# Mikubill/sketch2img

Hardware: AMD Instinct MI355X
Metric: sketch-guided images/sec whole-node, SD1.5 512px 50-step DDIM (higher is better)
Workload: dtype fp16

## Files before the change

### include/skg.h

```cpp
#ifndef SKG_H_
#define SKG_H_

#include <stddef.h>
#include <stdint.h>

#ifdef __cplusplus
extern "C" {
#endif

#define SKG_OK 0
#define SKG_E_BADARG (-1)
#define SKG_E_UNSUPPORTED (-2)
#define SKG_E_LAUNCH (-3)

#define SKG_ABI_VERSION 6
int skg_abi_version(void);
const char* skg_last_error(void);

#define SKG_EPI_RELU 1u
#define SKG_EPI_OUT_F32 2u
#define SKG_EPI_GEGLU 4u
#define SKG_EPI_BIAS_ROWS 8u

int skg_gemm_f16(const void* A, int lda, const void* B, int ldb, void* C, void* C_lo, int ldc, int M, int N, int K,
// ... 25 lines not shown
int skg_gemm_f16_rows(const void* A, int lda, const void* B, int ldb, void* C, int ldc, int M, int N, int K,
                      const void* bias, int seg_rows, int seg_stride, void* stream);
int skg_conv3x3_up2_f16(const void* X, int ldx, const void* Wpp, void* Y, void* Y_lo, int ldy, int rows, int IH, int IW, int Cin,
                        int Cout, int pair_in, const void* bias, void* stream);
int skg_conv3x3_sc_f16(const void* X, int ldx, const void* X2, int ldx2, int K2, const void* Wcat, void* Y, void* Y_lo, int ldy,
                       int rows, int IH, int IW, int Cin, int Cout, const void* bias, unsigned flags, float* gn_partial, int groups,
                       void* stream);
size_t skg_conv3x3_wino_v_bytes(int rows, int IH, int IW, int Cin);
int skg_conv3x3_wino_f16(const void* X, int ldx, const void* U, void* V, void* Y, void* Y_lo, int ldy, int rows, int IH, int IW,
                         int Cin, int Cout, const void* bias, const void* residual, const void* residual_lo, int ldr, unsigned flags,
                         void* stream);
int skg_groupnorm_wino_fwd(const void* X, int ldx, void* V, int rows, int IH, int IW, int C, int groups, float eps,
                           const void* gamma, const void* beta, int silu, float* stats, void* stream);
int skg_conv4x4s2_f16(const void* X, int ldx, const void* W16, void* Y, int ldy, int rows, int IH, int IW, int Cin,
                      int Cout, const void* bias, void* stream);


int skg_groupnorm_apply(const void* X, const void* X_lo, int ldx, void* Y, int ldy, int rows, int HW, int C, int groups,
                        const float* stats, const void* gamma, const void* beta, int silu, void* stream);
int skg_groupnorm_bwd(const void* X, int ldx, const void* dY, int lddy, void* dX, int lddx,
                      const void* residual, int ldr, int rows, int HW, int C, int groups,
                      const float* stats, const void* gamma, const void* beta, int silu,
                      float* partial, void* stream);

int skg_layernorm_fwd(const void* X, const void* X_lo, int ldx, void* Y, int ldy, int M, int C, const void* gamma,
                      const void* beta, float eps, float* stats, void* stream);
int skg_layernorm_bwd(const void* X, int ldx, const void* dY, int lddy, void* dX, int lddx,
                      const void* residual, int ldr, int M, int C, const void* gamma,
                      const float* stats, void* stream);

// ... 150 lines not shown
```

### sketch2img_amd/_lib.py

```python
from __future__ import annotations

import ctypes
import os

import torch

_HERE = os.path.dirname(os.path.abspath(__file__))
LIB_PATH = os.environ.get("SKG_LIB") or os.path.join(_HERE, "libskg.so")

ABI_VERSION = 6

SIGNATURES = {
    "skg_abi_version": ("i", ""),
    "skg_last_error": ("s", ""),
    "skg_gemm_f16": ("i", "pipippiiiipppifupiip"),
    "skg_conv3x3_up2_f16": ("i", "pipppiiiiiiipp"),
    "skg_conv3x3_sc_f16": ("i", "pipiipppiiiiiipupip"),
    "skg_conv4x4s2_f16": ("i", "pippiiiiiipp"),
    "skg_conv3x3_wino_v_bytes": ("z", "iiii"),
    "skg_conv3x3_wino_f16": ("i", "pippppiiiiiipppiup"),
    "skg_groupnorm_wino_fwd": ("i", "pipiiiiifppipp"),
    "skg_gemm_f16_rows": ("i", "pipipiiiipiip"),
    "skg_gemm_gn_fused": ("i", "iiiiiii"),
    "skg_gemm_f16_geglu_keep": ("i", "pipipipiiiipp"),
    "skg_ff_block_f16": ("i", "ppippiiiippfppppppippiipiip"),
    "skg_xattn_block_f16": ("i", "ppippiiiiiippfpppfpppipip"),
    "skg_gemm_variant": ("i", "iiiii"),
    "skg_set_workspace": ("i", "pzp"),
    "skg_conv3x3_f16": ("i", "pipppiiiiiiipppifupip"),
    "skg_groupnorm_scratch_floats": ("z", "ii"),
    "skg_groupnorm_stats": ("i", "piiiiifppp"),
    "skg_groupnorm_fwd": ("i", "ppippiiiiifppippp"),
    "skg_groupnorm_from_partial": ("i", "ppippiiiiiifppippipiip"),
# ... 105 lines not shown
```

### sketch2img_amd/csrc/gemm.hip

```cpp
#include "gemm_params.h"
#include <mutex>
#include <vector>

namespace {

constexpr int BM = 128;
constexpr int BK = 32;
constexpr int PITCH = 40;

template <int BN, int MODE>
__global__ __launch_bounds__(256) void gemm_kernel(const GemmParams p) {
  constexpr int WN = BN / 2;
  constexpr int NT = WN / 16;
  constexpr int MT = 4;
  constexpr int BPT = BN / 64;
  __shared__ __attribute__((aligned(16))) half_t As[2][BM * PITCH];
  __shared__ __attribute__((aligned(16))) half_t Bs[2][BN * PITCH];

  const int tid = threadIdx.x;
  const int lane = tid & 63;
  const int wave = tid >> 6;
  const int wm = wave >> 1, wn = wave & 1;
  const int g = lane >> 4, l16 = lane & 15;
  const int m0 = blockIdx.y * BM;
// ... 463 lines not shown
              skg_aligned(Y, 16) && (!bias || skg_aligned(bias, 8)));
  hipStream_t st = (hipStream_t)stream;
  GemmParams p{};
  p.A = (const half_t*)X; p.lda = ldx;
  p.B = (const half_t*)W16; p.ldb = 16 * Cin;
  p.C = Y; p.ldc = ldy; p.bias = (const half_t*)bias;
  p.N = Cout; p.K = 16 * Cin; p.alpha = 1.f; p.flags = 0;
  p.IH = IH; p.IW = IW; p.OH = IH / 2; p.OW = IW / 2; p.Cin = Cin; p.M = rows * p.OH * p.OW;
  p.ntaps = 16;
  ws_attach(p, st);
  if (!skg_gemm2_try_launch(p, MODE_S2, st)) return SKG_E_UNSUPPORTED;
  SKG_CHECK_LAUNCH("skg_conv4x4s2_f16");
  return SKG_OK;
}

static void conv_out_size(int mode, int IH, int IW, int* OH, int* OW) {
  const int up = (mode == SKG_CONV_UP2 || mode == SKG_CONV_S2T), dn = (mode == SKG_CONV_S2 || mode == SKG_CONV_S2A);
  *OH = up ? IH * 2 : dn ? IH / 2 : IH;
  *OW = up ? IW * 2 : dn ? IW / 2 : IW;
}

extern "C" int skg_conv3x3_f16(const void* X, int ldx, const void* Wp, void* Y, void* Y_lo, int ldy, int rows, int IH, int IW,
                               int Cin, int Cout, int mode, const void* bias, const void* residual, const void* residual_lo,
                               int ldr, float alpha, unsigned flags, float* gn_partial, int groups, void* stream) {
  int OH, OW;
  conv_out_size(mode, IH, IW, &OH, &OW);
  SKG_REQUIRE(!(flags & SKG_EPI_BIAS_ROWS) || bias);
  SKG_REQUIRE(!(Y_lo || residual_lo) || pair_args_ok(Y, Y_lo, ldy, residual, residual_lo, ldr, Cin, flags));
  SKG_REQUIRE(!gn_partial || (rows > 0 && OH > 0 && OW > 0 && skg_aligned(Y, 16) &&
                              gn_args_ok(gn_partial, rows * OH * OW, Cout, OH * OW, groups, ldy, flags)));
// ... 30 lines not shown
```

### sketch2img_amd/csrc/gemm2.hip

```cpp
#include "gemm_params.h"
#include <stdlib.h>

namespace {

constexpr int BK = 64;
constexpr unsigned OOB = 0x80000000u;

typedef __attribute__((address_space(3))) void* lds_ptr_t;

__device__ __forceinline__ void dma16(__amdgpu_buffer_rsrc_t rsrc, half_t* lds_wave_base, unsigned voff,
                                      unsigned soff) {
  __builtin_amdgcn_raw_ptr_buffer_load_lds(rsrc, (lds_ptr_t)lds_wave_base, 16, voff, soff, 0, 0);
}

template <int MASK, int N>
__device__ __forceinline__ void sgb() {
  if constexpr (N > 0) __builtin_amdgcn_sched_group_barrier(MASK, N, 0);
}
constexpr int SGB_MFMA = 0x008, SGB_VMEM = 0x010, SGB_DSREAD = 0x100;
template <int NT, int R, int V>
__device__ __forceinline__ void sched_group() {
  if constexpr (NT > 0) {
    sgb<SGB_MFMA, 1>();
    if constexpr (R > 0) {
// ... 95 lines not shown
}

template <int BM, int BN, int WGM, int WGN, int MODE, int NS, bool GNS, bool HILO, bool FIX, bool BROWS = false>
__device__ __forceinline__ void gemm2_body(const GemmParams& p, int tiles_n, int nwg, unsigned a_bytes, unsigned b_bytes,
                                           unsigned a_shift, int kt_per_split, float* __restrict__ ws) {
  constexpr int NW = WGM * WGN;
  constexpr int NTHR = NW * 64;
  constexpr int WM = BM / WGM;
  constexpr int WN = BN / WGN;
  constexpr int NT = WN / 16;
  constexpr int MT = WM / 16;
  constexpr int ACH = BM / 8 / NW;
  constexpr int BCH = BN / 8 / NW;
  static_assert(BM % (8 * NW) == 0 && BN % (8 * NW) == 0 && WM % 16 == 0 && WN % 16 == 0, "tile shape");
  constexpr int STAGE = (BM + BN) * BK;
  constexpr bool AFFINE = (MODE == MODE_DIRECT || MODE == MODE_S1 || MODE == MODE_S2 || MODE == MODE_S2A);
  __shared__ __attribute__((aligned(16))) half_t smem[NS * STAGE + 2 * BN];

  const int tid = threadIdx.x;
  const int lane = tid & 63;
  const int wave = __builtin_amdgcn_readfirstlane(tid >> 6);
  const int wm = wave / WGN, wn = wave - wm * WGN;
  const int g = lane >> 4, l16 = lane & 15;

  const __amdgpu_buffer_rsrc_t rA =
      __builtin_amdgcn_make_buffer_rsrc((void*)((const char*)p.A - a_shift), 0, a_bytes, 0x00020000);
  const __amdgpu_buffer_rsrc_t rB = __builtin_amdgcn_make_buffer_rsrc((void*)p.B, 0, b_bytes, 0x00020000);
  const __amdgpu_buffer_rsrc_t rA2 = __builtin_amdgcn_make_buffer_rsrc(
      (void*)(p.A2 ? p.A2 : p.A), 0, p.A2 ? ((unsigned)(p.M - 1) * (unsigned)p.lda2 + (unsigned)p.K2) * 2u : 0u, 0x00020000);
  const int KT1 = (MODE == MODE_S1 && p.K2) ? (p.K - p.K2) / BK : (1 << 30);

// ... 6 lines not shown
    g_phase[vb][7] = __builtin_amdgcn_s_getreg((31 << 11) | 20);
    g_phase[vb][5] = __builtin_amdgcn_s_getreg((31 << 11) | 6);
  }
#endif
  int lid;
  {
    const int bid = vb;
    const int xcd = bid & 7, idx = bid >> 3;
    const int q = nwg >> 3, r = nwg & 7;
    lid = (xcd < r ? xcd * (q + 1) : r * (q + 1) + (xcd - r) * q) + idx;
  }
  const int ntiles = ws ? nwg / ((p.K / BK + kt_per_split - 1) / kt_per_split) : nwg;
  const int split = lid / ntiles;
  lid -= split * ntiles;
  int ph = p.up2 ? p.up2 - 1 : 0;
  if (p.up2 == 5) {
    const int per = ntiles >> 2;
    ph = lid / per;
    lid -= ph * per;
  }
  int tile_m = lid / tiles_n;
  int tile_n = lid - tile_m * tiles_n;
  if (const int gn = (p.flags >> 20) & 0xf) {
    const int G = ((p.flags >> 24) & 0xf) ? (int)((p.flags >> 24) & 0xf) : 8;
    const int per = ntiles / G, tmb = (ntiles / tiles_n) / (G / gn), tnb = tiles_n / gn;
    const int xr = lid / per, r = lid - xr * per;
    const int xm = xr / gn, xn = xr - xm * gn;
    const int rm = r / tnb;
    tile_m = xm * tmb + rm;
    tile_n = xn * tnb + (r - rm * tnb);
  }
  const int m0 = tile_m * BM, n0 = tile_n * BN;

  const int lr = lane >> 3;
  const int lq = lane & 7;
// ... 7 lines not shown
    const int r = (j * NW + wave) * 8 + lr;
    const unsigned pk = (unsigned)(lq ^ ((r >> 1) & 7)) * 16u;
    const int m = m0 + r;
    const bool ok = m < p.M;
    const int mm = ok ? m : 0;
    a_mask[j] = 0; a_oy[j] = a_ox[j] = 0; a_img[j] = 0;
    if (MODE == MODE_DIRECT) {
      a_voff[j] = ok ? (unsigned)mm * (unsigned)p.lda * 2u + pk : OOB;
    } else {
      const int ohw = p.OH * p.OW;
      const int b = mm / ohw;
      if (j == 0) smp0 = b;
      const int rr = mm - b * ohw;
      const int oy = rr / p.OW, ox = rr - oy * p.OW;
      const unsigned img = (unsigned)b * (unsigned)(p.IH * p.IW);
      if (MODE == MODE_S1 || MODE == MODE_S2 || MODE == MODE_S2A) {
        const int cy = MODE == MODE_S1 ? oy : 2 * oy + (MODE == MODE_S2A), cx = MODE == MODE_S1 ? ox : 2 * ox + (MODE == MODE_S2A);
        a_voff[j] = ok ? ((img + (unsigned)(cy * p.IW + cx)) * (unsigned)p.lda) * 2u + pk : OOB;
        unsigned mk = 0;
        if (MODE == MODE_S2 && p.ntaps == 16) {
#pragma unroll
          for (int t = 0; t < 16; ++t) {
            const int iy = cy + (t >> 2) - 1, ix = cx + (t & 3) - 1;
            if (ok && iy >= 0 && iy < p.IH && ix >= 0 && ix < p.IW) mk |= 1u << t;
          }
        } else {
#pragma unroll
          for (int t = 0; t < 9; ++t) {
            const int iy = cy + t / 3 - 1, ix = cx + t % 3 - 1;
            if (ok && iy >= 0 && iy < p.IH && ix >= 0 && ix < p.IW) mk |= 1u << t;
          }
        }
// ... 28 lines not shown
        d.va[j] = (live && m0 + r < p.M) ? (unsigned)(m0 + r) * (unsigned)p.lda2 * 2u + pk : OOB;
      }
#pragma unroll
      for (int j = 0; j < BCH; ++j) d.vb[j] = live ? b_voff[j] : OOB;
      d.soa = (unsigned)(kt - KT1) * (BK * 2u);
      d.sob = (unsigned)kt * (BK * 2u);
      return d;
    }
    const int k0 = kt * BK;
    unsigned soff = (unsigned)k0 * 2u;
    int tap = 0, ky = 0, kx = 0, c0 = 0;
    unsigned kb = (unsigned)k0;
    if (MODE != MODE_DIRECT) {
      int ti;
      if (tap_minor) {
        const int nt = p.ntaps ? p.ntaps : 9;
        const int cb = kt / nt;
        ti = kt - cb * nt;
        c0 = cb * BK;
      } else {
        ti = k0 / p.Cin;
        c0 = k0 - ti * p.Cin;
      }
      kb = (unsigned)(ti * p.Cin + c0);
      if (MODE == MODE_S2 && p.ntaps == 16) {
        tap = ti;
        ky = ti >> 2;
        kx = ti & 3;
      } else {
        const unsigned tapmap = p.up2 == 5 ? (unsigned)((ph >> 1) * 3 + (ph & 1)) * 0x1111u + 0x4310u : p.tapmap;
        tap = p.ntaps ? (int)((tapmap >> (4 * ti)) & 0xfu) : ti;
        ky = tap / 3;
        kx = tap - ky * 3;
      }
      const int ca = (p.a_wrap && c0 >= p.a_wrap) ? c0 - p.a_wrap : c0;
      soff = (unsigned)((ky * p.IW + kx) * p.lda + ca) * 2u;
    }
#pragma unroll
    for (int j = 0; j < ACH; ++j) {
      unsigned v;
// ... 108 lines not shown
    }
#endif
#pragma unroll
    for (int ks = 0; ks < 2; ++ks)
#pragma unroll
      for (int i = 0; i < MT; ++i)
#pragma unroll
        for (int j = 0; j < NT; ++j)
          acc[i][j] = __builtin_amdgcn_mfma_f32_16x16x32_f16(wf[ks][j], xf[ks][i], acc[i][j], 0, 0, 0);
#ifdef SKG_LAB
    if (!(p.flags & 0x2000u))
#endif
    sched_plan<MT, NT, ND>();
  };

  const int kt_begin = split * kt_per_split;
  const int KT = min(p.K / BK, kt_begin + kt_per_split);
  float bias_r = 0.f;
  if constexpr (!BROWS) {
    const half_t* bias_t = p.bias;
    if constexpr (MODE != MODE_DIRECT) bias_t += __builtin_amdgcn_readfirstlane(smp0) * p.bias_pitch;
    bias_r = (tid < BN && p.bias && n0 + tid < p.N) ? (float)bias_t[n0 + tid] : 0.f;
  }
  SKG_PH(1);
  {
    const DmaStep d0 = dma_prepare(kt_begin, true);
#pragma unroll
    for (int i = 0; i < ND; ++i) dma_one(d0, 0, i);
  }
  if constexpr (NS == 2) {
    for (int kt = kt_begin; kt < KT; kt += 2) {
      asm volatile("s_waitcnt vmcnt(0)" ::: "memory");
// ... 24 lines not shown
        }
      }
    }
  }
  asm volatile("s_waitcnt vmcnt(0)" ::: "memory");

  SKG_PH(2);
#ifdef SKG_PHASES
  if ((tid & 63) == 0 && vb < (1 << 15)) g_phase[vb][12 + (tid >> 6)] = __builtin_readcyclecounter();
#endif
  const bool stream_out = p.flags & 0x800u;
  const bool relu = p.flags & SKG_EPI_RELU;
  const bool f32out = p.flags & SKG_EPI_OUT_F32;
  if (ws) {
    float* slab = ws + (size_t)split * p.M * p.N;
#pragma unroll
    for (int i = 0; i < MT; ++i) {
      const int m = m0 + wm * WM + i * 16 + l16;
      if (m >= p.M) continue;
#pragma unroll
      for (int j = 0; j < NT; ++j) {
        const int n = n0 + wn * WN + j * 16 + g * 4;
        if (n < p.N) {
          *reinterpret_cast<float4_t*>(slab + (size_t)m * p.N + n) = acc[i][j];
        }
      }
    }
    if constexpr (FIX) {
      __shared__ unsigned s_ticket;
      const int splits = nwg / ntiles;
// ... 448 lines not shown
#endif

__global__ __launch_bounds__(256) void splitk_reduce_kernel(const GemmParams p, const float* __restrict__ ws,
                                                            int splits) {
  const int N4 = p.N >> 2;
  const size_t total = (size_t)p.M * N4;
  const size_t slab = (size_t)p.M * p.N;
  for (size_t i = (size_t)blockIdx.x * 256 + threadIdx.x; i < total; i += (size_t)gridDim.x * 256) {
    const size_t m = i / N4;
    const int n = (int)(i - m * N4) * 4;
    float4_t v = *reinterpret_cast<const float4_t*>(ws + m * p.N + n);
    for (int s = 1; s < splits; ++s) v += *reinterpret_cast<const float4_t*>(ws + s * slab + m * p.N + n);
    splitk_epilogue(p, v, m, n);
  }
}


struct SplitTuning { int target, smax, ns; };
inline SplitTuning read_split_tuning() {
  auto geti = [](const char* n, int dflt) { const char* e = getenv(n); return e ? atoi(e) : dflt; };
  SplitTuning t{geti("SKG_SPLIT_TARGET", 512), geti("SKG_MAX_SPLITS", 8), geti("SKG_SPLIT_NS", 3 )};
  t.target = t.target < 1 ? 1 : t.target > 4096 ? 4096 : t.target;
  t.smax = t.smax < 1 ? 1 : t.smax > 64 ? 64 : t.smax;
  t.ns = t.ns <= 2 ? 2 : t.ns >= 4 ? 4 : 3;
  return t;
}
inline SplitTuning split_tuning() {
#ifdef SKG_LAB
  return read_split_tuning();
#else
// ... 64 lines not shown
  if (!p.gn_partial || p.gn_groups <= 0 || p.gn_hw <= 0 || !eligible(p, mode)) return false;
  if (p.flags & (SKG_EPI_OUT_F32 | SKG_EPI_GEGLU)) return false;
  const bool hilo = p.c_lo || p.res_lo;
  TileCfg t = pick_tile(p.M, p.N, p.K);
  if (hilo && t.bm == 256) t = TileCfg{128, 160};
  if (t.bm != 128 || t.bn != 160) return false;
  if (p.M % 128 != 0 || p.N % 160 != 0 || p.gn_hw % 128 != 0 || p.M % p.gn_hw != 0 || p.N % p.gn_groups != 0) return false;
  const int cpg = p.N / p.gn_groups;
  if ((cpg & 1) || 160 % cpg != 0) return false;
  if (p.ldc % 8 != 0 || (reinterpret_cast<uintptr_t>(p.C) & 15) != 0) return false;
  if (p.res && (p.ldr % 8 != 0 || (reinterpret_cast<uintptr_t>(p.res) & 15) != 0)) return false;
  const long ntiles = (long)(p.M / 128) * (p.N / 160);
  return pick_splits(ntiles, p.K / BK, (size_t)p.M * p.N * 4, p.ws, p.ws_bytes) == 1;
}

template <int BM, int BN, int WGM, int WGN, int MODE>
void launch_cfg(const GemmParams& p_in, hipStream_t st) {
  GemmParams p = p_in;
  const size_t out_bytes = (size_t)p.M * ((p.flags & SKG_EPI_GEGLU) ? p.N / 2 : p.N) * ((p.flags & SKG_EPI_OUT_F32) ? 4 : 2);
  static const bool tap_major = getenv("SKG_TAP_MAJOR") != nullptr;
  if (MODE != MODE_DIRECT && !tap_major) p.flags |= 0x1000u;
#ifdef SKG_LAB
  if (MODE != MODE_DIRECT && getenv("SKG_GLUE_PROBE")) p.flags |= 0x2000u;
#endif
  static const char* smb = getenv("SKG_STREAM_MB");
  if (out_bytes >= (smb ? (size_t)atoi(smb) << 20 : STREAM_OUT_BYTES)) p.flags |= 0x800u;
#ifdef SKG_LAB
  static const int direct_epi = getenv("SKG_DIRECT_EPI") ? atoi(getenv("SKG_DIRECT_EPI")) : 0;
  const bool direct_ok = direct_epi && !(p.flags & (SKG_EPI_GEGLU | SKG_EPI_OUT_F32)) && !p.c_lo && !p.res_lo && !p.gn_partial && !p.up2 &&
                         !p.seg_rows && !p.ntaps && !p.bias_pitch && p.N % BN == 0 && p.ldc % 8 == 0 && skg_aligned(p.C, 16) &&
                         (!p.res || (p.ldr % 8 == 0 && skg_aligned(p.res, 16))) && (!p.bias || skg_aligned(p.bias, 16)) &&
                         (direct_epi == 1 || p.K <= 640);
#else
  constexpr bool direct_ok = false;
#endif
  const int tiles_n = skg_cdiv(p.N, BN);
  const int ntiles = skg_cdiv(p.M, BM) * tiles_n * (p.up2 == 5 ? 4 : 1);
  unsigned long long a, b, s;
  operand_bytes(p, MODE, a, b, s);
  const int KT = p.K / BK;
  int splits = (BM == 128 && !(p.flags & SKG_EPI_GEGLU) && !p.up2 && !p.seg_rows) ? pick_splits(ntiles, KT, (size_t)p.M * p.N * 4, p.ws, p.ws_bytes) : 1;
  if (p.wino) splits = p.wino;
  constexpr int NTHR = WGM * WGN * 64;
  if (BM == 128 && BN == 160 && splits == 1 && gn_fusable(p, MODE)) p.flags |= SKG_FLAG_GN_STATS;
  if (p.bias_pitch && (p.gn_hw % BM != 0 || (p.flags & SKG_EPI_OUT_F32) || p.ldc % 8 != 0 || !skg_aligned(p.C, 16) || (p.res && (p.ldr % 8 != 0 || !skg_aligned(p.res, 16)))))
    p.flags |= SKG_FLAG_BIAS_PER_ROW;
  if (direct_ok && splits == 1) p.flags |= 0x10000u;
  const int ns_eff = splits > 1 ? skg_cdiv(KT, skg_cdiv(KT, splits)) : 1;
  const int G = (8 % ns_eff == 0) ? 8 / ns_eff : 0;
  if (G >= 2 && ntiles % G == 0 && p.up2 != 5) {
    static const bool off = getenv("SKG_NO_XGRID") != nullptr;
    const int tiles_m = ntiles / tiles_n;
    const double a_mb = (double)p.M * (MODE == MODE_DIRECT ? p.K : p.Cin) * 2.0, w_mb = (double)p.N * p.K * 2.0;
    int best = 1;
    double cost = a_mb + G * w_mb;
    for (int gn = 2; gn <= G; gn *= 2) {
      if (tiles_n % gn != 0 || tiles_m % (G / gn) != 0) continue;
      const double c = gn * a_mb + (G / gn) * w_mb;
      if (c < 0.9 * cost) { cost = c; best = gn; }
    }
    static const char* force_gn = getenv("SKG_XGRID_GN");
    if (force_gn) {
      const int gn = atoi(force_gn);
      best = (gn >= 1 && gn <= G && G % gn == 0 && tiles_n % gn == 0 && tiles_m % (G / gn) == 0) ? gn : 1;
    }
// ... 17 lines not shown
      const int sns = split_tuning().ns;
      if (ntiles * ns <= 256 && per >= 4 && sns >= 3) {
        deep = true;
        if (sns >= 4)
          hipLaunchKernelGGL((gemm2_kernel<BM, BN, WGM, WGN, MODE, 4, false, false>), dim3(ntiles * ns), dim3(NTHR), 0, st, p, tiles_n, ntiles * ns,
                             (unsigned)a, (unsigned)b, (unsigned)s, per, p.ws);
        else
          hipLaunchKernelGGL((gemm2_kernel<BM, BN, WGM, WGN, MODE, 3, false, false>), dim3(ntiles * ns), dim3(NTHR), 0, st, p, tiles_n, ntiles * ns,
                             (unsigned)a, (unsigned)b, (unsigned)s, per, p.ws);
      }
    }
    if (!deep)
      hipLaunchKernelGGL((gemm2_kernel<BM, BN, WGM, WGN, MODE>), dim3(persistent_grid(ntiles * ns, NTHR)), dim3(NTHR),
                         0, st, p, tiles_n, ntiles * ns, (unsigned)a, (unsigned)b, (unsigned)s, per, p.ws);
    if (p.wino) return;
    size_t blocks = ((size_t)p.M * (p.N / 4) + 255) / 256;
    hipLaunchKernelGGL(splitk_reduce_kernel, dim3((unsigned)(blocks > 2048 ? 2048 : blocks)), dim3(256), 0, st, p,
                       (const float*)p.ws, ns);
    return;
  }
  const bool hilo = p.c_lo || p.res_lo;
  constexpr bool HILO_OK = BM == 128 && (MODE == MODE_DIRECT || MODE == MODE_S1 || MODE == MODE_S2 || MODE == MODE_UP2);
  const bool gns = (p.flags & SKG_FLAG_GN_STATS) != 0;
  if constexpr (BM == 128 && MODE != MODE_DIRECT) {
    if (p.flags & SKG_FLAG_BIAS_PER_ROW) {
      if constexpr (HILO_OK) {
        if (hilo) {
          hipLaunchKernelGGL((gemm2_kernel<BM, BN, WGM, WGN, MODE, 2, false, true, true>), dim3(ntiles), dim3(NTHR), 0, st, p, tiles_n, ntiles,
                             (unsigned)a, (unsigned)b, (unsigned)s, KT, (float*)nullptr);
          return;
// ... 18 lines not shown
        if (ns == 6 && KT >= 7) { G2_LAUNCH(6, false, false); return; }
      }
    }
#endif
    if (!off && KT >= 4 && (BN == 64 || ntiles <= 256)) {
      if constexpr (BN == 160) {
        if (gns) {
          if (hilo) G2_LAUNCH(3, true, true); else G2_LAUNCH(3, true, false);
          return;
        }
      }
      if (hilo) G2_LAUNCH(3, false, true); else G2_LAUNCH(3, false, false);
      return;
    }
  }
#ifdef SKG_PHASES
  static const char* solo = getenv("SKG_SOLO");
  if (solo) {
    hipLaunchKernelGGL((gemm2_kernel<BM, BN, WGM, WGN, MODE>), dim3(ntiles), dim3(NTHR), 48 * 1024, st,
                       p, tiles_n, ntiles, (unsigned)a, (unsigned)b, (unsigned)s, KT, (float*)nullptr);
    return;
  }
#endif
  if constexpr (HILO_OK) {
    if (hilo) {
      if constexpr (BN == 160 && MODE != MODE_UP2) {
        if (gns) { G2_LAUNCH(2, true, true); return; }
      }
      G2_LAUNCH(2, false, true);
      return;
// ... 27 lines not shown
  const TileCfg t = pick_tile(M, N, K);
  const int KT = K / BK;
  const long ntiles = (long)skg_cdiv(M, t.bm) * skg_cdiv(N, t.bn);
  const int splits = t.bm == 128 ? pick_splits(ntiles, KT, (size_t)M * N * 4, ws_bytes ? (const float*)1 : nullptr, ws_bytes) : 1;
  bool three = t.bm == 128 && (t.bn == 160 || t.bn == 64) && (mode == MODE_DIRECT || mode == MODE_S1) &&
               !getenv("SKG_NO_NS3") && KT >= 4 && (t.bn == 64 || ntiles <= 256) && splits == 1;
  if (splits > 1 && t.bm == 128 && t.bn == 160 && (mode == MODE_DIRECT || mode == MODE_S1)) {
    const int per = skg_cdiv(KT, splits), ns = skg_cdiv(KT, per);
    three = ntiles * ns <= 256 && per >= 4 && split_tuning().ns >= 3;
  }
  return t.bn + (three ? 10000 : 0);
}

bool skg_gemm2_fuses_gn(const GemmParams& p, int mode) { return gn_fusable(p, mode); }

void skg_splitk_reduce_launch(const GemmParams& p, const float* ws, int splits, hipStream_t st) {
  size_t blocks = ((size_t)p.M * (p.N / 4) + 255) / 256;
  hipLaunchKernelGGL(splitk_reduce_kernel, dim3((unsigned)(blocks > 2048 ? 2048 : blocks)), dim3(256), 0, st, p, ws, splits);
}

bool skg_gemm2_try_launch(const GemmParams& p, int mode, hipStream_t st) {
  if (!eligible(p, mode)) return false;
  if (p.wino &&
      (mode != MODE_DIRECT || p.wino != 16 || (p.K / BK) % 16 != 0 || !p.ws || (size_t)16 * p.M * p.N * 4 > p.ws_bytes || p.gn_partial ||
       p.seg_rows || p.up2 || p.aux || (p.flags & (SKG_EPI_GEGLU | SKG_EPI_OUT_F32))))
    return false;
  if (p.seg_rows &&
      (mode != MODE_DIRECT || p.res || p.gn_partial || p.c_lo || p.res_lo || p.aux || (p.flags & (SKG_EPI_GEGLU | SKG_EPI_OUT_F32)) ||
       p.ldc % 8 != 0 || (reinterpret_cast<uintptr_t>(p.C) & 15) != 0))
    return false;
  if ((p.ntaps || p.up2) &&
      ((p.ntaps == 16 ? (mode != MODE_S2 || p.up2 || p.c_lo) : mode != MODE_S1) || p.res || p.gn_partial || p.res_lo || (p.flags & (SKG_EPI_GEGLU | SKG_EPI_OUT_F32)) ||
       p.ldc % 8 != 0 || (reinterpret_cast<uintptr_t>(p.C) & 15) != 0 || p.M % (p.OH * p.OW) != 0))
    return false;
  if ((p.c_lo || p.res_lo) &&
      ((p.flags & (SKG_EPI_GEGLU | SKG_EPI_OUT_F32)) || p.aux || p.ldc % 8 != 0 ||
       (mode != MODE_DIRECT && mode != MODE_S1 && mode != MODE_S2 && mode != MODE_UP2) || (mode == MODE_UP2 && p.gn_partial) ||
       (reinterpret_cast<uintptr_t>(p.C) & 15) != 0 || (p.c_lo && (reinterpret_cast<uintptr_t>(p.c_lo) & 15) != 0) ||
       ((p.res || p.res_lo) && p.ldr % 8 != 0) || (p.res && (reinterpret_cast<uintptr_t>(p.res) & 15) != 0) ||
       (p.res_lo && (reinterpret_cast<uintptr_t>(p.res_lo) & 15) != 0)))
    return false;
  if ((p.flags & SKG_EPI_GEGLU) && ((p.flags & SKG_EPI_OUT_F32) || p.res || p.ldc % 8 != 0 ||
                                     (reinterpret_cast<uintptr_t>(p.C) & 15) != 0))
    return false;
  switch (mode) {
    case MODE_DIRECT: launch_mode<MODE_DIRECT>(p, st); break;
    case MODE_S1: launch_mode<MODE_S1>(p, st); break;
    case MODE_S2: launch_mode<MODE_S2>(p, st); break;
    case MODE_UP2: launch_mode<MODE_UP2>(p, st); break;
    case MODE_S2T: launch_mode<MODE_S2T>(p, st); break;
    case MODE_S2A: launch_mode<MODE_S2A>(p, st); break;
    default: return false;
  }
  return true;
}

#ifdef SKG_PHASES
extern "C" int skg_debug_phases(void* host_out, int nblocks) {
  return (int)hipMemcpyFromSymbol(host_out, HIP_SYMBOL(g_phase), (size_t)nblocks * 16 * sizeof(unsigned long long));
}
#endif
```

### sketch2img_amd/csrc/gemm_params.h

```cpp
#pragma once
#include "common.h"

enum { MODE_DIRECT = 0, MODE_S1 = 1, MODE_S2 = 2, MODE_UP2 = 3, MODE_S2T = 4, MODE_S2A = 5 };

struct GemmParams {
  const half_t* A; int lda;
  const half_t* B; int ldb;
  void* C; int ldc;
  const half_t* bias;
  const half_t* res; int ldr;
  int M, N, K;
  float alpha; unsigned flags;
  int IH, IW, OH, OW, Cin;
  float* gn_partial; int gn_hw, gn_groups;
  half_t* aux; int ldaux;
  const half_t* res_lo; half_t* c_lo;
  int ntaps; unsigned tapmap; int up2;
  int a_wrap;
  int seg_rows, seg_stride;
  const half_t* A2; int lda2, K2;
  int wino;
  float* ws; size_t ws_bytes;
  unsigned* ws_cnt;
  int bias_pitch;
// ... 24 lines not shown
```

### sketch2img_amd/ops.py

```python
from __future__ import annotations

import ctypes
import threading
from typing import List, Optional, Sequence, Tuple

import torch

from ._lib import SkgError, SkgTap, check, lib

EPI_RELU, EPI_OUT_F32, EPI_GEGLU, EPI_BIAS_ROWS = 1, 2, 4, 8
CONV_S1, CONV_S2, CONV_UP2, CONV_S2T, CONV_S2A = 0, 1, 2, 3, 4
ATTN_CAUSAL, ATTN_ROWV, ATTN_RESIDENT_KV = 1, 2, 4


_workspace = {}
_workspace_lock = threading.Lock()
WORKSPACE_BYTES = 128 << 20
_capture_owner = None


def _stream() -> int:
    st = torch.cuda.current_stream()
    key = (st.device.index, st.cuda_stream)
    if key not in _workspace:
# ... 208 lines not shown
    if keep_from is not None:
        Mk = M - keep_from
        dev = Xh.device
        st = torch.empty(Mk, 2, device=dev, dtype=torch.float32)
        q = torch.empty(Mk, C, device=dev, dtype=torch.float16)
        o = torch.empty(Mk, C, device=dev, dtype=torch.float16)
        lse = torch.empty(Mk // HW, heads, HW, device=dev, dtype=torch.float32)
    check(lib.skg_xattn_block_f16(_p(Xh), _p(X.lo) if pair else None, _ld(Xh), _p(Yh), _p(Yl), _ld(Yh), M, HW, C, heads, Nkv,
                                  _p(gamma), _p(beta), eps, _p(wpack), _p(kvpack), _p(bias_out), scale, _p(st), _p(q), _p(o), C,
                                  _p(lse), keep_from or 0, _stream()), "skg_xattn_block_f16")
    return out if keep_from is None else (out, st, q, o, lse)


def conv3x3(X: torch.Tensor, Wp: torch.Tensor, rows: int, IH: int, IW: int, mode: int = CONV_S1,
            out: Optional[torch.Tensor] = None, *, bias=None, residual=None, alpha: float = 1.0,
            relu: bool = False, gn_groups: Optional[int] = None, out_lo=None, residual_lo=None):
    Cin = X.shape[1]
    Cout = Wp.shape[0]
    brows = _bias_rows_flag(bias, rows, Cout)
    _f16(X, Wp, bias, residual, out_lo, residual_lo)
    assert Wp.shape[1] == 9 * Cin and Wp.is_contiguous() and X.shape[0] == rows * IH * IW
    if mode == CONV_S1:
        OH, OW = IH, IW
    elif mode in (CONV_S2, CONV_S2A):
        OH, OW = IH // 2, IW // 2
    else:
        OH, OW = IH * 2, IW * 2
    if out is None:
        out = torch.empty(rows * OH * OW, Cout, device=X.device, dtype=torch.float16)
    assert out_lo is None or _ld(out_lo) == _ld(out)
    assert residual_lo is None or residual is None or _ld(residual_lo) == _ld(residual)
    r_any = residual if residual is not None else residual_lo
    part = GNPartial(rows, OH * OW, gn_groups, X.device) if gn_groups is not None else None
    check(lib.skg_conv3x3_f16(_p(X), _ld(X), _p(Wp), _p(out), _p(out_lo), _ld(out), rows, IH, IW, Cin, Cout, mode,
                              _p(bias), _p(residual), _p(residual_lo), _ld(r_any) if r_any is not None else 0,
                              alpha, (EPI_RELU if relu else 0) | brows, _p(part.buf) if part is not None else None, gn_groups or 0,
                              _stream()), "skg_conv3x3_f16")
    return out if part is None else (out, part)


def conv3x3_small(X: torch.Tensor, Wp: torch.Tensor, B: int, IH: int, IW: int, stride: int = 1, out: Optional[torch.Tensor] = None, *,
                  bias=None, silu: bool = False):
    if X.dtype == torch.float32:
        if X.dim() != 4 or tuple(X.shape) != (B, 3, IH, IW) or not X.is_contiguous() or not X.is_cuda:
            raise ValueError(f"conv3x3_small: a contiguous fp32 CUDA picture [{B}, 3, {IH}, {IW}] expected, got {tuple(X.shape)}")
        Cin, ldx = 3, 0
    else:
# ... 791 lines not shown
```

### sketch2img_amd/unet.py

```python
from __future__ import annotations

import functools
import math
import os
from dataclasses import dataclass, field
from typing import Callable, Dict, List, Optional, Sequence, Tuple

import torch

from . import ops
from .config import UNetConfig, up_block_plan
from .packs import (CIN_PAD, COUT_PAD, CTX_PAD, EPS_SEED_LD, _h, _pad_vec, pack_conv, pack_conv_dgrad,
                    pack_conv_up2, pack_conv_up2_dgrad, pack_conv_up2_hilo, pack_conv_wino, pack_ff_block, pack_xattn_kv,
                    pack_xattn_weights)

_GN_FROM_PRODUCER = os.environ.get("SKG_GN_PRODUCER", "1") != "0"
_GN_CONCAT = os.environ.get("SKG_GN_CONCAT", "1") != "0"
_FF_BLOCK = os.environ.get("SKG_FF_BLOCK", "1") != "0"
_XATTN_BLOCK = os.environ.get("SKG_XATTN_BLOCK", "1") != "0"
_FF_KEEP = os.environ.get("SKG_FF_KEEP", "1") != "0"
_XATTN_HEADS = (8,) if os.environ.get("SKG_XATTN_D64", "1") == "0" else (8, 5)
_RESIDENT_KV_BUILT = frozenset({(40, 10), (40, 15), (64, 10), (64, 15), (80, 10), (80, 15), (160, 10)})
_RESIDENT_KV = _RESIDENT_KV_BUILT if os.environ.get("SKG_RESIDENT_KV", "0") == "1" else frozenset()
_XATTN_KEEP = os.environ.get("SKG_XATTN_KEEP", "1") != "0"
# ... 17 lines not shown


def _side(sz: Tuple[int, int]):
    return sz[0] if sz[0] == sz[1] else sz


UP2_POLYPHASE = os.environ.get("SKG_UP2_POLY", "1") != "0"
HP_UP_TRIPLE = os.environ.get("SKG_HP_UP_TRIPLE", "0") != "0"
HP_NORM_PAIRS = tuple(n for n in os.environ.get(
    "SKG_HP_NORM_PAIRS", "up_blocks.{last}.resnets.0.norm2,up_blocks.{last}.resnets.1.norm1,up_blocks.{last}.resnets.1.norm2,"
                         "up_blocks.{last}.resnets.2.norm1,up_blocks.{last}.resnets.2.norm2,up_blocks.{last}.attentions.0.norm,"
                         "up_blocks.{last}.attentions.1.norm,up_blocks.{last}.attentions.2.norm").split(",") if n)
HP_PLAIN_LEVELS = int(os.environ.get("SKG_HP_PLAIN_LEVELS", "1"))
UP2_SMALL_MAPS = os.environ.get("SKG_UP2_SMALL", "1") != "0"
UP2_DGRAD = os.environ.get("SKG_UP2_DGRAD", "1") != "0"


@dataclass
class Stash:
    res: Dict[str, dict] = field(default_factory=dict)
    tr: Dict[str, dict] = field(default_factory=dict)
    misc: dict = field(default_factory=dict)
    rows: int = 0
    first: int = 0

    def suffix(self, key: str, v: Optional[torch.Tensor], unit: int) -> Optional[torch.Tensor]:
        if v is None:
            return None
        S, (n, rem) = self.rows - self.first, divmod(v.shape[0], unit)
        if rem or not S <= n <= self.rows:
# ... 916 lines not shown
            if 0 < i <= 3:
                dh = add(dh, tap_grads[6 + i - 1])
        dh = add(dh, tap_grads[5])
        dh = self._res_bwd("mid_block.resnets.1", dh, S, stash.res["mid_block.resnets.1"])
        dh = add(dh, tap_grads[3])
        dh = self._tr_bwd("mid_block.attentions.0", dh, S, stash.tr["mid_block.attentions.0"], inject_bwd)
        dh = add(dh, tap_grads[4])
        dh = self._res_bwd("mid_block.resnets.0", dh, S, stash.res["mid_block.resnets.0"])
        k = n_skips - 1
        for i in range(nb - 1, -1, -1):
            if i < nb - 1:
                dh = add(dh, gskip[k]); k -= 1
                if i < 3:
                    dh = add(dh, tap_grads[i])
                p = f"down_blocks.{i}.downsamplers.0.conv"
                dh = ops.conv3x3(dh, W[p + ".weight:T"], S, *cur, ops.CONV_S2T)
                cur = _dbl(cur)
            for j in range(lpb - 1, -1, -1):
                dh = add(dh, gskip[k]); k -= 1
                if i < nb - 1:
                    dh = self._tr_bwd(f"down_blocks.{i}.attentions.{j}", dh, S,
                                      stash.tr[f"down_blocks.{i}.attentions.{j}"], inject_bwd)
                    if stop_early and i == 0 and j == 0:
                        return None
                dh = self._res_bwd(f"down_blocks.{i}.resnets.{j}", dh, S, stash.res[f"down_blocks.{i}.resnets.{j}"])
        dh = add(dh, gskip[0])
        return ops.conv3x3(dh, W["conv_in.weight:T"], S, *sz)
```

Baseline: 6.028.

## Add polyphase gather kernel for stride-2 transposed conv in downsampler backward

```diff
diff --git a/include/skg.h b/include/skg.h
--- a/include/skg.h
+++ b/include/skg.h
@@ -63,6 +63,8 @@
                            const void* gamma, const void* beta, int silu, float* stats, void* stream);
 int skg_conv4x4s2_f16(const void* X, int ldx, const void* W16, void* Y, int ldy, int rows, int IH, int IW, int Cin,
                       int Cout, const void* bias, void* stream);
+int skg_conv3x3_s2t_f16(const void* dY, int ldx, const void* WT, void* dX, int ldy, int rows, int OH, int OW, int Cin, int Cout,
+                        void* stream);
 
 
 int skg_groupnorm_apply(const void* X, const void* X_lo, int ldx, void* Y, int ldy, int rows, int HW, int C, int groups,
diff --git a/sketch2img_amd/_lib.py b/sketch2img_amd/_lib.py
--- a/sketch2img_amd/_lib.py
+++ b/sketch2img_amd/_lib.py
@@ -17,6 +17,7 @@
     "skg_conv3x3_up2_f16": ("i", "pipppiiiiiiipp"),
     "skg_conv3x3_sc_f16": ("i", "pipiipppiiiiiipupip"),
     "skg_conv4x4s2_f16": ("i", "pippiiiiiipp"),
+    "skg_conv3x3_s2t_f16": ("i", "pippiiiiiip"),
     "skg_conv3x3_wino_v_bytes": ("z", "iiii"),
     "skg_conv3x3_wino_f16": ("i", "pippppiiiiiipppiup"),
     "skg_groupnorm_wino_fwd": ("i", "pipiiiiifppipp"),
diff --git a/sketch2img_amd/csrc/gemm.hip b/sketch2img_amd/csrc/gemm.hip
--- a/sketch2img_amd/csrc/gemm.hip
+++ b/sketch2img_amd/csrc/gemm.hip
@@ -501,6 +501,25 @@
   return SKG_OK;
 }
 
+extern "C" int skg_conv3x3_s2t_f16(const void* dY, int ldx, const void* WT, void* dX, int ldy, int rows, int OH, int OW, int Cin,
+                                   int Cout, void* stream) {
+  SKG_REQUIRE(dY && WT && dX && rows > 0 && OH > 0 && OW > 0 && Cin > 0 && Cout > 0);
+  SKG_REQUIRE(Cin % 32 == 0 && Cout % 8 == 0 && ldx % 8 == 0 && ldx >= Cin && ldy % 4 == 0 && ldy >= Cout);
+  SKG_REQUIRE(skg_aligned(dY, 16) && skg_aligned(WT, 16) && skg_aligned(dX, 8));
+  if ((OH & 1) || (OW & 1) || Cin % 64 != 0) return SKG_E_UNSUPPORTED;
+  hipStream_t st = (hipStream_t)stream;
+  GemmParams p{};
+  p.A = (const half_t*)dY; p.lda = ldx; p.B = (const half_t*)WT; p.ldb = 9 * Cin; p.C = dX; p.ldc = ldy;
+  p.N = Cout; p.K = 9 * Cin; p.alpha = 1.f; p.flags = 0;
+  p.IH = OH / 2; p.IW = OW / 2; p.Cin = Cin;
+  ws_attach(p, st);
+  p.OH = p.IH; p.OW = p.IW; p.M = rows * p.IH * p.IW; p.gn_hw = p.IH * p.IW;
+  p.ntaps = 4; p.up2 = 6;
+  if (!skg_gemm2_try_launch(p, MODE_S2P, st)) return SKG_E_UNSUPPORTED;
+  SKG_CHECK_LAUNCH("skg_conv3x3_s2t_f16");
+  return SKG_OK;
+}
+
 static void conv_out_size(int mode, int IH, int IW, int* OH, int* OW) {
   const int up = (mode == SKG_CONV_UP2 || mode == SKG_CONV_S2T), dn = (mode == SKG_CONV_S2 || mode == SKG_CONV_S2A);
   *OH = up ? IH * 2 : dn ? IH / 2 : IH;
diff --git a/sketch2img_amd/csrc/gemm2.hip b/sketch2img_amd/csrc/gemm2.hip
--- a/sketch2img_amd/csrc/gemm2.hip
+++ b/sketch2img_amd/csrc/gemm2.hip
@@ -133,7 +133,7 @@
   constexpr int BCH = BN / 8 / NW;
   static_assert(BM % (8 * NW) == 0 && BN % (8 * NW) == 0 && WM % 16 == 0 && WN % 16 == 0, "tile shape");
   constexpr int STAGE = (BM + BN) * BK;
-  constexpr bool AFFINE = (MODE == MODE_DIRECT || MODE == MODE_S1 || MODE == MODE_S2 || MODE == MODE_S2A);
+  constexpr bool AFFINE = (MODE == MODE_DIRECT || MODE == MODE_S1 || MODE == MODE_S2 || MODE == MODE_S2A || MODE == MODE_S2P);
   __shared__ __attribute__((aligned(16))) half_t smem[NS * STAGE + 2 * BN];
 
   const int tid = threadIdx.x;
@@ -170,11 +170,15 @@
   const int split = lid / ntiles;
   lid -= split * ntiles;
   int ph = p.up2 ? p.up2 - 1 : 0;
-  if (p.up2 == 5) {
+  if (p.up2 == 5 || MODE == MODE_S2P) {
     const int per = ntiles >> 2;
     ph = lid / per;
     lid -= ph * per;
-  }
+    if (MODE == MODE_S2P) ph = 3 - ph;
+  }
+  const int s2p_nt = (1 + (ph >> 1)) * (1 + (ph & 1));
+  const unsigned s2p_in = ph == 0 ? 0x4u : ph == 1 ? 0x54u : ph == 2 ? 0x74u : 0x8754u;
+  const unsigned s2p_w = ph == 0 ? 0x4u : ph == 1 ? 0x53u : ph == 2 ? 0x71u : 0x8620u;
   int tile_m = lid / tiles_n;
   int tile_n = lid - tile_m * tiles_n;
   if (const int gn = (p.flags >> 20) & 0xf) {
@@ -212,8 +216,9 @@
       const int rr = mm - b * ohw;
       const int oy = rr / p.OW, ox = rr - oy * p.OW;
       const unsigned img = (unsigned)b * (unsigned)(p.IH * p.IW);
-      if (MODE == MODE_S1 || MODE == MODE_S2 || MODE == MODE_S2A) {
-        const int cy = MODE == MODE_S1 ? oy : 2 * oy + (MODE == MODE_S2A), cx = MODE == MODE_S1 ? ox : 2 * ox + (MODE == MODE_S2A);
+      if (MODE == MODE_S1 || MODE == MODE_S2 || MODE == MODE_S2A || MODE == MODE_S2P) {
+        constexpr bool S1C = MODE == MODE_S1 || MODE == MODE_S2P;
+        const int cy = S1C ? oy : 2 * oy + (MODE == MODE_S2A), cx = S1C ? ox : 2 * ox + (MODE == MODE_S2A);
         a_voff[j] = ok ? ((img + (unsigned)(cy * p.IW + cx)) * (unsigned)p.lda) * 2u + pk : OOB;
         unsigned mk = 0;
         if (MODE == MODE_S2 && p.ntaps == 16) {
@@ -272,7 +277,7 @@
     if (MODE != MODE_DIRECT) {
       int ti;
       if (tap_minor) {
-        const int nt = p.ntaps ? p.ntaps : 9;
+        const int nt = MODE == MODE_S2P ? s2p_nt : p.ntaps ? p.ntaps : 9;
         const int cb = kt / nt;
         ti = kt - cb * nt;
         c0 = cb * BK;
@@ -280,8 +285,12 @@
         ti = k0 / p.Cin;
         c0 = k0 - ti * p.Cin;
       }
-      kb = (unsigned)(ti * p.Cin + c0);
-      if (MODE == MODE_S2 && p.ntaps == 16) {
+      kb = (unsigned)((MODE == MODE_S2P ? (int)((s2p_w >> (4 * ti)) & 0xfu) : ti) * p.Cin + c0);
+      if (MODE == MODE_S2P) {
+        tap = (int)((s2p_in >> (4 * ti)) & 0xfu);
+        ky = tap / 3;
+        kx = tap - ky * 3;
+      } else if (MODE == MODE_S2 && p.ntaps == 16) {
         tap = ti;
         ky = ti >> 2;
         kx = ti & 3;
@@ -420,8 +429,25 @@
     sched_plan<MT, NT, ND>();
   };
 
-  const int kt_begin = split * kt_per_split;
-  const int KT = min(p.K / BK, kt_begin + kt_per_split);
+  int kt_begin = split * kt_per_split;
+  int KT = min(p.K / BK, kt_begin + kt_per_split);
+  if constexpr (MODE == MODE_S2P) {
+    auto below = [&](int x) {
+      const int cbs = p.Cin / BK;
+      const int q = tap_minor ? x / 9 : x / cbs, r = tap_minor ? x - q * 9 : x - q * cbs;
+      const int t = tap_minor ? r : q;
+      int n = 0, live = 0;
+#pragma unroll
+      for (int ti = 0; ti < 4; ++ti) {
+        const int w = (int)((s2p_w >> (4 * ti)) & 0xfu);
+        n += (ti < s2p_nt && w < t);
+        live |= (ti < s2p_nt && w == t);
+      }
+      return tap_minor ? q * s2p_nt + n : n * cbs + (live ? r : 0);
+    };
+    kt_begin = below(kt_begin);
+    KT = below(KT);
+  }
   float bias_r = 0.f;
   if constexpr (!BROWS) {
     const half_t* bias_t = p.bias;
@@ -476,6 +502,7 @@
   const bool f32out = p.flags & SKG_EPI_OUT_F32;
   if (ws) {
     float* slab = ws + (size_t)split * p.M * p.N;
+    if constexpr (MODE == MODE_S2P) slab = ws + ((size_t)split * 4 + ph) * p.M * p.N;
 #pragma unroll
     for (int i = 0; i < MT; ++i) {
       const int m = m0 + wm * WM + i * 16 + l16;
@@ -954,6 +981,21 @@
     splitk_epilogue(p, v, m, n);
   }
 }
+__global__ __launch_bounds__(256) void splitk_reduce_s2p_kernel(const GemmParams p, const float* __restrict__ ws, int splits) {
+  const int N4 = p.N >> 2;
+  const size_t total = (size_t)4 * p.M * N4;
+  const size_t slab = (size_t)4 * p.M * p.N;
+  const int hw = p.OH * p.OW;
+  for (size_t i = (size_t)blockIdx.x * 256 + threadIdx.x; i < total; i += (size_t)gridDim.x * 256) {
+    const size_t r = i / N4;
+    const int n = (int)(i - r * N4) * 4;
+    float4_t v = *reinterpret_cast<const float4_t*>(ws + r * p.N + n);
+    for (int s = 1; s < splits; ++s) v += *reinterpret_cast<const float4_t*>(ws + s * slab + r * p.N + n);
+    const int ph = (int)(r / (size_t)p.M), m = (int)(r - (size_t)ph * p.M);
+    const int img = m / hw, rr = m - img * hw, y = rr / p.OW, x = rr - y * p.OW;
+    splitk_epilogue(p, v, (size_t)img * 4 * hw + (size_t)(2 * y + (ph >> 1)) * (2 * p.OW) + 2 * x + (ph & 1), n);
+  }
+}
 
 
 struct SplitTuning { int target, smax, ns; };
@@ -1048,6 +1090,13 @@
   return pick_splits(ntiles, p.K / BK, (size_t)p.M * p.N * 4, p.ws, p.ws_bytes) == 1;
 }
 
+inline int s2t_gather_splits(const GemmParams& p) {
+  const int M = 4 * p.M;
+  const TileCfg t = pick_tile(M, p.N, p.K);
+  if (t.bm != 128) return 1;
+  return pick_splits((long)skg_cdiv(M, 128) * skg_cdiv(p.N, t.bn), p.K / BK, (size_t)M * p.N * 4, p.ws, p.ws_bytes);
+}
+
 template <int BM, int BN, int WGM, int WGN, int MODE>
 void launch_cfg(const GemmParams& p_in, hipStream_t st) {
   GemmParams p = p_in;
@@ -1069,12 +1118,13 @@
   constexpr bool direct_ok = false;
 #endif
   const int tiles_n = skg_cdiv(p.N, BN);
-  const int ntiles = skg_cdiv(p.M, BM) * tiles_n * (p.up2 == 5 ? 4 : 1);
+  const int ntiles = skg_cdiv(p.M, BM) * tiles_n * (p.up2 >= 5 ? 4 : 1);
   unsigned long long a, b, s;
   operand_bytes(p, MODE, a, b, s);
   const int KT = p.K / BK;
   int splits = (BM == 128 && !(p.flags & SKG_EPI_GEGLU) && !p.up2 && !p.seg_rows) ? pick_splits(ntiles, KT, (size_t)p.M * p.N * 4, p.ws, p.ws_bytes) : 1;
   if (p.wino) splits = p.wino;
+  if constexpr (MODE == MODE_S2P && BM == 128) splits = s2t_gather_splits(p);
   constexpr int NTHR = WGM * WGN * 64;
   if (BM == 128 && BN == 160 && splits == 1 && gn_fusable(p, MODE)) p.flags |= SKG_FLAG_GN_STATS;
   if (p.bias_pitch && (p.gn_hw % BM != 0 || (p.flags & SKG_EPI_OUT_F32) || p.ldc % 8 != 0 || !skg_aligned(p.C, 16) || (p.res && (p.ldr % 8 != 0 || !skg_aligned(p.res, 16)))))
@@ -1082,7 +1132,7 @@
   if (direct_ok && splits == 1) p.flags |= 0x10000u;
   const int ns_eff = splits > 1 ? skg_cdiv(KT, skg_cdiv(KT, splits)) : 1;
   const int G = (8 % ns_eff == 0) ? 8 / ns_eff : 0;
-  if (G >= 2 && ntiles % G == 0 && p.up2 != 5) {
+  if (G >= 2 && ntiles % G == 0 && p.up2 < 5) {
     static const bool off = getenv("SKG_NO_XGRID") != nullptr;
     const int tiles_m = ntiles / tiles_n;
     const double a_mb = (double)p.M * (MODE == MODE_DIRECT ? p.K : p.Cin) * 2.0, w_mb = (double)p.N * p.K * 2.0;
@@ -1130,6 +1180,11 @@
       hipLaunchKernelGGL((gemm2_kernel<BM, BN, WGM, WGN, MODE>), dim3(persistent_grid(ntiles * ns, NTHR)), dim3(NTHR),
                          0, st, p, tiles_n, ntiles * ns, (unsigned)a, (unsigned)b, (unsigned)s, per, p.ws);
     if (p.wino) return;
+    if constexpr (MODE == MODE_S2P) {
+      const size_t blocks4 = ((size_t)4 * p.M * (p.N / 4) + 255) / 256;
+      hipLaunchKernelGGL(splitk_reduce_s2p_kernel, dim3((unsigned)(blocks4 > 2048 ? 2048 : blocks4)), dim3(256), 0, st, p, (const float*)p.ws, ns);
+      return;
+    }
     size_t blocks = ((size_t)p.M * (p.N / 4) + 255) / 256;
     hipLaunchKernelGGL(splitk_reduce_kernel, dim3((unsigned)(blocks > 2048 ? 2048 : blocks)), dim3(256), 0, st, p,
                        (const float*)p.ws, ns);
@@ -1178,6 +1233,10 @@
       return;
     }
   }
+  if constexpr (MODE == MODE_S2P && BN == 160) {
+    static const bool off = getenv("SKG_NO_NS3") != nullptr;
+    if (!off && ntiles <= 256) { G2_LAUNCH(3, false, false); return; }
+  }
 #ifdef SKG_PHASES
   static const char* solo = getenv("SKG_SOLO");
   if (solo) {
@@ -1235,6 +1294,7 @@
 
 bool skg_gemm2_fuses_gn(const GemmParams& p, int mode) { return gn_fusable(p, mode); }
 
+
 void skg_splitk_reduce_launch(const GemmParams& p, const float* ws, int splits, hipStream_t st) {
   size_t blocks = ((size_t)p.M * (p.N / 4) + 255) / 256;
   hipLaunchKernelGGL(splitk_reduce_kernel, dim3((unsigned)(blocks > 2048 ? 2048 : blocks)), dim3(256), 0, st, p, ws, splits);
@@ -1251,9 +1311,11 @@
        p.ldc % 8 != 0 || (reinterpret_cast<uintptr_t>(p.C) & 15) != 0))
     return false;
   if ((p.ntaps || p.up2) &&
-      ((p.ntaps == 16 ? (mode != MODE_S2 || p.up2 || p.c_lo) : mode != MODE_S1) || p.res || p.gn_partial || p.res_lo || (p.flags & (SKG_EPI_GEGLU | SKG_EPI_OUT_F32)) ||
+      ((p.ntaps == 16 ? (mode != MODE_S2 || p.up2 || p.c_lo) : p.up2 == 6 ? (mode != MODE_S2P || p.c_lo || p.bias || p.a_wrap) : mode != MODE_S1) ||
+       p.res || p.gn_partial || p.res_lo || (p.flags & (SKG_EPI_GEGLU | SKG_EPI_OUT_F32)) ||
        p.ldc % 8 != 0 || (reinterpret_cast<uintptr_t>(p.C) & 15) != 0 || p.M % (p.OH * p.OW) != 0))
     return false;
+  if (mode == MODE_S2P && (p.up2 != 6 || p.K != 9 * p.Cin || p.OH != p.IH || p.OW != p.IW)) return false;
   if ((p.c_lo || p.res_lo) &&
       ((p.flags & (SKG_EPI_GEGLU | SKG_EPI_OUT_F32)) || p.aux || p.ldc % 8 != 0 ||
        (mode != MODE_DIRECT && mode != MODE_S1 && mode != MODE_S2 && mode != MODE_UP2) || (mode == MODE_UP2 && p.gn_partial) ||
@@ -1271,6 +1333,7 @@
     case MODE_UP2: launch_mode<MODE_UP2>(p, st); break;
     case MODE_S2T: launch_mode<MODE_S2T>(p, st); break;
     case MODE_S2A: launch_mode<MODE_S2A>(p, st); break;
+    case MODE_S2P: launch_mode<MODE_S2P>(p, st); break;
     default: return false;
   }
   return true;
diff --git a/sketch2img_amd/csrc/gemm_params.h b/sketch2img_amd/csrc/gemm_params.h
--- a/sketch2img_amd/csrc/gemm_params.h
+++ b/sketch2img_amd/csrc/gemm_params.h
@@ -1,7 +1,7 @@
 #pragma once
 #include "common.h"
 
-enum { MODE_DIRECT = 0, MODE_S1 = 1, MODE_S2 = 2, MODE_UP2 = 3, MODE_S2T = 4, MODE_S2A = 5 };
+enum { MODE_DIRECT = 0, MODE_S1 = 1, MODE_S2 = 2, MODE_UP2 = 3, MODE_S2T = 4, MODE_S2A = 5, MODE_S2P = 6 };
 
 struct GemmParams {
   const half_t* A; int lda;
diff --git a/sketch2img_amd/ops.py b/sketch2img_amd/ops.py
--- a/sketch2img_amd/ops.py
+++ b/sketch2img_amd/ops.py
@@ -246,7 +246,7 @@
 
 def conv3x3(X: torch.Tensor, Wp: torch.Tensor, rows: int, IH: int, IW: int, mode: int = CONV_S1,
             out: Optional[torch.Tensor] = None, *, bias=None, residual=None, alpha: float = 1.0,
-            relu: bool = False, gn_groups: Optional[int] = None, out_lo=None, residual_lo=None):
+            relu: bool = False, gn_groups: Optional[int] = None, out_lo=None, residual_lo=None, polyphase: bool = True):
     Cin = X.shape[1]
     Cout = Wp.shape[0]
     brows = _bias_rows_flag(bias, rows, Cout)
@@ -263,6 +263,14 @@
     assert out_lo is None or _ld(out_lo) == _ld(out)
     assert residual_lo is None or residual is None or _ld(residual_lo) == _ld(residual)
     r_any = residual if residual is not None else residual_lo
+    if (mode == CONV_S2T and polyphase and bias is None and r_any is None and alpha == 1.0 and not relu and gn_groups is None
+            and out_lo is None):
+        _f16(out)
+        rc = lib.skg_conv3x3_s2t_f16(_p(X), _ld(X), _p(Wp), _p(out), _ld(out), rows, OH, OW, Cin, Cout, _stream())
+        if rc == 0:
+            return out
+        if rc != -2:
+            check(rc, "skg_conv3x3_s2t_f16")
     part = GNPartial(rows, OH * OW, gn_groups, X.device) if gn_groups is not None else None
     check(lib.skg_conv3x3_f16(_p(X), _ld(X), _p(Wp), _p(out), _p(out_lo), _ld(out), rows, IH, IW, Cin, Cout, mode,
                               _p(bias), _p(residual), _p(residual_lo), _ld(r_any) if r_any is not None else 0,
diff --git a/sketch2img_amd/unet.py b/sketch2img_amd/unet.py
--- a/sketch2img_amd/unet.py
+++ b/sketch2img_amd/unet.py
@@ -55,6 +55,7 @@
 HP_PLAIN_LEVELS = int(os.environ.get("SKG_HP_PLAIN_LEVELS", "1"))
 UP2_SMALL_MAPS = os.environ.get("SKG_UP2_SMALL", "1") != "0"
 UP2_DGRAD = os.environ.get("SKG_UP2_DGRAD", "1") != "0"
+S2T_POLYPHASE = os.environ.get("SKG_S2T_POLY", "1") != "0"
 
 
 @dataclass
@@ -1001,7 +1002,7 @@
                 if i < 3:
                     dh = add(dh, tap_grads[i])
                 p = f"down_blocks.{i}.downsamplers.0.conv"
-                dh = ops.conv3x3(dh, W[p + ".weight:T"], S, *cur, ops.CONV_S2T)
+                dh = ops.conv3x3(dh, W[p + ".weight:T"], S, *cur, ops.CONV_S2T, polyphase=S2T_POLYPHASE)
                 cur = _dbl(cur)
             for j in range(lpb - 1, -1, -1):
                 dh = add(dh, gskip[k]); k -= 1
```

Result: no change. 6.051 (median of 6 runs) (+0.4%).
